# Gabisanth/MaximumAreaCoverageOptimization.jl

Hardware: AMD Instinct MI355X
Metric: MADS objective evals/sec (N UAVs × M fire cells), 1/2/4/8 MI355X (higher is better)
Workload: dtype f64

## Files before the change

maximumareacoverageoptimization.jl_amd/csrc/k_prep.h:

```cpp
#pragma once

#include <hip/hip_runtime.h>
#include <stdint.h>

#include "predicate.h"
#include "k_common.h"

#pragma clang fp contract(off)

namespace mac {


struct PenArgs {
    const double* rmax;
    const double* prev;
    const double* dlimT;
    const double* dlim;
    double tan_half_fov;
};

__device__ __forceinline__ double pen_threshold(const PenArgs& pa, int i)
{
    if (!pa.prev) return 0.0;
    return pa.dlimT ? pa.dlimT[i] : dlim_threshold(pa.dlim[i]);
}

__device__ __forceinline__ double pen_term(double x2, double y2, double R2, int i, int N,
                                           const PenArgs& pa, double T3)
{
    if (pa.prev) {
        const double x1 = pa.prev[i], y1 = pa.prev[N + i], z1 = pa.prev[2 * N + i] / pa.tan_half_fov;
        const double z2 = R2 / pa.tan_half_fov;
        const double ddx = x1 - x2, ddy = y1 - y2, ddz = z1 - z2;
        const double s = ddx * ddx + ddy * ddy + ddz * ddz;
        if (s > T3) return -1.0;
    }
    return pa.rmax ? __builtin_fabs(R2 - pa.rmax[i]) : 0.0;
}

__host__ __device__ __forceinline__ bool diag_rejects(double v, double b, double p, int q,
                                                      double tan_half_fov, double T3)
{
    bool all = true;
#pragma unroll
    for (int sg = 0; sg < 2; ++sg) {
        const double c = sg == 0 ? v + b : v - b;
        double d;
        if (q < 2) {
            d = p - c;
        } else {
            const double z1 = p / tan_half_fov, z2 = c / tan_half_fov;
            d = z1 - z2;
        }
        const double sq = d * d;
        all = all && sq > T3;
    }
    return all;
}


__host__ __device__ __forceinline__ uint64_t splitmix_at(uint64_t state, uint64_t idx)
{
    uint64_t z = state + idx * 0x9E3779B97F4A7C15ull;
    z = (z ^ (z >> 30)) * 0xBF58476D1CE4E5B9ull;
    z = (z ^ (z >> 27)) * 0x94D049BB133111EBull;
    return z ^ (z >> 31);
}

__host__ __device__ __forceinline__ double splitmix_uniform_at(uint64_t state, uint64_t idx)
{
    return (double)(splitmix_at(state, idx) >> 11) * (1.0 / 9007199254740992.0);
}

__host__ __device__ __forceinline__ double ltmads_entry(uint64_t state, int64_t n, int64_t b,
                                                        int64_t r, int64_t c)
{
    if (r < c) return 0.0;
    if (r == c) return (splitmix_uniform_at(state, (uint64_t)r + 1) < 0.5 ? -1.0 : 1.0) * (double)b;
    const int64_t lo = -b + 1, span = 2 * b - 1;
    const double u = splitmix_uniform_at(state, (uint64_t)(n + 1 + r * (r - 1) / 2 + c));
    return (double)(lo + (int64_t)__builtin_floor(u * (double)span));
}

struct MadsState {
    double f;
    int64_t it;
    int ell;
    int skip;
    unsigned long long feas;
    int64_t skipped;
    int64_t succ;
};

struct CandSrc {
    const double* cands;
    int ldc;
    const uint32_t* keysP;
    const float* keysT;
    int ldk;
    const double* xinc;
    const int* rp;
    const int* cp;
    uint64_t state;
    int64_t b;
    int k0;
    int np;
    const MadsState* mst;
    const int16_t* ltri;
    double delta;
    int route_five;
    __device__ __forceinline__ bool resolve(bool any_poll = false)
    {
        if (!mst) return true;
        const int e = mst->ell;
        if (e < 0 || (!any_poll && mst->skip)) return false;
        b = (int64_t)1 << e;
        return true;
    }
    __host__ __device__ __forceinline__ int polled(int N) const { return np ? np : 3 * N; }
    __device__ __forceinline__ double entry(int n, int r, int c) const
    {
        if (ltri) return r < c ? 0.0 : delta * (double)ltri[(int64_t)r * (r + 1) / 2 + c];
        return ltmads_entry(state, n, b, r, c);
    }
    __device__ __forceinline__ double get_full(int kl, int v, int N) const
    {
        if (cands) return cands[(int64_t)kl * ldc + v];
        const int n = 3 * N;
        const int k = kl + k0;
        const int kk = k < n ? k : k - n;
        const double d = entry(n, rp[v], cp[kk]);
        return k < n ? xinc[v] + d : xinc[v] - d;
    }
    __device__ __forceinline__ double get(int kl, int v, int N) const
    {
        if (cands) return cands[(int64_t)kl * ldc + v];
        const int n = polled(N);
        const int k = kl + k0;
        const int kk = k < n ? k : k - n;
        const bool held = v >= n;
// ... 40 lines not shown
    float* keysT;
    int ldk;
    double4* pd;
    uint8_t* dead8;
    MadsState* mst_w;
    unsigned long long* feas;
    int* lreset;
    const uint8_t* mask8;
};

template <int NC, class Cand>
__device__ __forceinline__ uint32_t prep_masked(const uint8_t* mask8, int K, Cand cand)
{
    uint32_t m = 0u;
    if (mask8) {
#pragma unroll
        for (int c = 0; c < NC; ++c) {
            const int k = cand(c);
            if (k < K && mask8[k] == 0) m |= 1u << c;
        }
    }
    return m;
}

constexpr int kPrepCX = 6;

constexpr uint32_t kKeyEsc = 0x200u << 22;
__device__ __forceinline__ bool key_int(double v, double b, double lim, int& d)
{
    const double f = v - b;
    if (!(f >= -lim && f <= lim)) return false;
    d = (int)f;
    return (double)d == f && __builtin_bit_cast(uint64_t, b + (double)d) == __builtin_bit_cast(uint64_t, v);
}
__device__ __forceinline__ uint32_t key_pack(int dx, int dy, int dr)
{
    return ((uint32_t)dx & 0x7FFu) | (((uint32_t)dy & 0x7FFu) << 11) | (((uint32_t)dr & 0x3FFu) << 22);
}
__device__ __forceinline__ void key_unpack(uint32_t p, float& x, float& y, float& r)
{
    x = (float)((int)(p << 21) >> 21);
    y = (float)((int)(p << 10) >> 21);
    r = (float)((int)p >> 22);
}

__device__ __forceinline__ bool partial_range(double a, double b, double m, double g0, double invS,
                                              int n, int& lo, int& hi)
{
    const double ulo = (a - g0) * invS;
    const double uhi = (b - g0) * invS;
    const double err = (m + __builtin_fabs(g0)) * invS * 1e-14 + 1e-9;
    const double flo = __builtin_floor(ulo - err);
    const double fhi = __builtin_floor(uhi + err);
    if (!(flo == flo) || !(fhi == fhi)) { lo = 0; hi = n - 1; return true; }
    if (fhi < 0.0 || flo > (double)(n - 1)) return false;
    lo = flo < 0.0 ? 0 : (int)flo;
    hi = fhi > (double)(n - 1) ? n - 1 : (int)fhi;
    return true;
}

__host__ __device__ inline int range_shift(int n)
{
    int s = 0;
    while (((n - 1) >> s) > 0xFFFE) ++s;
    return s;
}
__device__ __forceinline__ uint32_t range_pack(bool any, int lo, int hi, int s)
{
    return any ? (uint32_t)(lo >> s) | ((uint32_t)(hi >> s) << 16) : 0xFFFFu;
}
__device__ __forceinline__ void range_unpack(uint32_t lo16, uint32_t hi16, int s, int n, int& lo, int& hi)
{
    lo = (int)(lo16 << s);
    hi = min((int)(((hi16 + 1) << s) - 1), n - 1);
}

#ifdef MAC_DIAG
__device__ uint64_t g_diag_prep[64 * 16];
#define MAC_PREP_STAMP_T(q, t) if (threadIdx.x == (t) && cw < 64 && (q) < 16) g_diag_prep[16 * cw + (q)] = __builtin_amdgcn_s_memrealtime()
#else
#define MAC_PREP_STAMP_T(q, t)
#endif
#define MAC_PREP_STAMP(q) MAC_PREP_STAMP_T(q, 0)

__device__ __forceinline__ void lds_barrier()
{
    asm volatile("s_waitcnt lgkmcnt(0)\n\ts_barrier" ::: "memory");
}

template <int PC>
struct PrepLds {
    double term[PC][kPrepU + 2];
    int wbad[kPrepU / kWave][PC];
    uint32_t wbadm[kPrepU / kWave];
    int wrej[kPrepU / kWave];
    double dred[kPrepU / kWave][4];
};

template <bool kMat, int PC>
__device__ __forceinline__ void prep_block(const PrepArgs& a, int cw, unsigned char* lds)
{
    constexpr int NC = PC;
    PrepLds<NC>& L = *reinterpret_cast<PrepLds<NC>*>(lds);
    auto& term = L.term;
    auto& wbad = L.wbad;
    auto& wbadm = L.wbadm;
    auto& wrej = L.wrej;
    auto& dred = L.dred;
    const int N = a.N, K = a.K;
    const int u = threadIdx.x, lane = u & (kWave - 1), wid = u / kWave;
    const int k0 = cw * PC;
    const int np = a.src.polled(N);
    auto cand = [&](int c) { return a.pair ? (c < 4 ? 4 * cw + c : np + 4 * cw + c - 4) : k0 + c; };
    const bool obj = a.vp != nullptr;
    const PenArgs& pa = a.pa;
    MAC_PREP_STAMP(0);
    double acc = 0.0;
    bool bad = false;
    uint32_t mdead = 0u;
    if constexpr (!kMat) mdead = prep_masked<NC>(obj ? a.mask8 : nullptr, K, cand);
    const bool masked = !kMat && a.mask8 != nullptr;
    const bool excl = obj && (pa.prev || masked) && (a.prec || a.pd) && a.skip_failed && N <= kPrepU;
    double dmx = -__builtin_inf(), dmy = -__builtin_inf(), dmr = -__builtin_inf();
    double dml = -__builtin_inf();
    uint32_t dead = 0u;
    for (int ib = 0; ib < N; ib += kPrepU) {
        const int nb = min(kPrepU, N - ib);
        const int i = ib + u;
        const bool iv = u < nb;
        const int ii = min(i, N - 1);
        double v[NC][3];
        if (!kMat && PC == 8 && a.pair) {
#pragma unroll
            for (int c = 0; c < 4; ++c) {
                const int col = 4 * cw + c;
#pragma unroll
                for (int q = 0; q < 3; ++q) {
                    const int vv = q * N + ii;
                    if (q == 2 && 2 * N >= np) {
                        v[c][q] = v[c + 4][q] = a.src.xinc[vv];
                        continue;
                    }
                    const double d = a.src.entry(np, a.src.rp[vv], a.src.cp[col]);
                    v[c][q] = a.src.xinc[vv] + d;
                    v[c + 4][q] = a.src.xinc[vv] - d;
                }
            }
        } else {
#pragma unroll
            for (int c = 0; c < NC; ++c) {
                const int k = min(cand(c), K - 1);
#pragma unroll
                for (int q = 0; q < 3; ++q) {
                    if constexpr (kMat) v[c][q] = a.src.cands[(int64_t)k * a.src.ldc + q * N + ii];
                    else v[c][q] = a.src.get(k, q * N + ii, N);
                }
            }
        }
        double base[3] = {0.0, 0.0, 0.0};
        if (a.keysP) {
#pragma unroll
            for (int q = 0; q < 3; ++q) {
                if constexpr (kMat) base[q] = a.src.cands[q * N + ii];
                else base[q] = a.src.get(0, q * N + ii, N);
            }
        }
// ... 122 lines not shown
        }
        if ((a.prec || a.keysP) && iv) {
            double xa = __builtin_inf(), xb = -__builtin_inf(), ya = __builtin_inf(), yb = -__builtin_inf();
            double xm = 0.0, ym = 0.0, est = 0.0;
            bool any = false;
#pragma unroll
            for (int c = 0; c < NC; ++c) {
                if (!a.prec) break;
                const double x = v[c][0], y = v[c][1], r = v[c][2];
                if (cand(c) < K && !((dead >> c) & 1u) && r > 0.0 && __builtin_isfinite(x) &&
                    __builtin_isfinite(y)) {
                    any = true;
                    xa = fmin(xa, x - r);
                    xb = fmax(xb, x + r);
                    ya = fmin(ya, y - r);
                    yb = fmax(yb, y + r);
                    xm = fmax(xm, __builtin_fabs(x) + r);
                    ym = fmax(ym, __builtin_fabs(y) + r);
                    const double e = 2.0 * r * a.g.invS + 1.0;
                    est += e * e;
                }
            }
            bool kb = false;
            if (a.keysP) {
                uint32_t pk[NC];
#pragma unroll
                for (int c = 0; c < NC; ++c) {
                    int dx = 0, dy = 0, dr = 0;
                    const bool packs = key_int(v[c][0], base[0], 1023.0, dx) &&
                                       key_int(v[c][1], base[1], 1023.0, dy) &&
                                       key_int(v[c][2], base[2], 511.0, dr);
                    pk[c] = packs ? key_pack(dx, dy, dr) : kKeyEsc;
                    if (!packs) {
#pragma unroll
                        for (int q = 0; q < 3; ++q) {
                            const float f = (float)(v[c][q] - base[q]);
                            kb |= !((dead >> c) & 1u) && __builtin_bit_cast(uint64_t, base[q] + (double)f) != __builtin_bit_cast(uint64_t, v[c][q]);
                            a.keysT[(int64_t)(q * N + i) * a.ldk + cand(c)] = f;
                        }
                    }
                }
                uint32_t* const krow = a.keysP + (int64_t)i * a.ldk;
#pragma unroll
                for (int h = 0; h < PC / 4; ++h)
                    *reinterpret_cast<uint4*>(krow + cand(4 * h)) =
                        make_uint4(pk[4 * h], pk[4 * h + 1], pk[4 * h + 2], pk[4 * h + 3]);
            }
            if (a.prec) {
                int x0 = 0, x1 = -1, y0 = 0, y1 = -1;
                any = any && partial_range(xa, xb, xm, a.g.gx0, a.g.invS, a.g.nTx, x0, x1) &&
                      partial_range(ya, yb, ym, a.g.gy0, a.g.invS, a.g.nTy, y0, y1);
                a.prec[(int64_t)cw * N + i] =
                    make_int4((int)range_pack(any, x0, x1, range_shift(a.g.nTx)),
                              (int)range_pack(any, y0, y1, range_shift(a.g.nTy)),
                              __builtin_bit_cast(int, (float)est), kb ? 1 : 0);
            }
        }
        MAC_PREP_STAMP(3 + 3 * (ib / kPrepU));
        if (obj && ib + kPrepU < N) lds_barrier();
    }
    if (obj && u < NC && cand(u) < K) {
        a.vp[cand(u)] = bad ? __builtin_inf() : acc * a.penalty;
        if (a.dead8) a.dead8[cand(u)] = excl && bad ? 1 : 0;
    }
    if (obj && a.feas && wid == 0) {
        const uint64_t ok = __ballot(u < NC && cand(u) < K && !bad);
        if (lane == 0 && ok) atomicAdd(a.feas, (unsigned long long)__popcll(ok));
    }
    if (a.pd) {
        lds_barrier();
        if (u == 0) {
            double4 m = make_double4(dred[0][0], dred[0][1], dred[0][2], dred[0][3]);
            for (int q = 1; q < kPrepU / kWave; ++q) {
                m.x = fmax(m.x, dred[q][0]);
                m.y = fmax(m.y, dred[q][1]);
                m.z = fmax(m.z, dred[q][2]);
                m.w = fmax(m.w, dred[q][3]);
            }
            a.pd[cw] = m;
        }
    }
}

template <bool kGen>
__device__ __forceinline__ void prep_block_x(const PrepArgs& a, int cw, unsigned char* lds)
{
    constexpr int PC = kPrepCX, NC = kGen ? kPrepCX : kPrepCX + 1, NW = kPrepU / kWave;
    PrepLds<kPrepCX + 1>& L = *reinterpret_cast<PrepLds<kPrepCX + 1>*>(lds);
    auto& term = L.term;
    auto& wbad = L.wbad;
    auto& wbadm = L.wbadm;
    auto& wrej = L.wrej;
    auto& dred = L.dred;
    const int N = a.N, K = a.K;
    const int u = threadIdx.x, lane = u & (kWave - 1), wid = u / kWave;
    const bool fw = wid == NW;
    const int k0 = cw * PC;
    const int n3 = 3 * N;
    auto cand = [&](int c) {
        if constexpr (kGen) return c < 3 ? 3 * cw + c : n3 + 3 * cw + c - 3;
        else return c < PC ? k0 + c : a.xbase + cw;
    };
    const bool obj = a.vp != nullptr;
    const PenArgs& pa = a.pa;
    uint32_t mdead = 0u;
    if constexpr (kGen) mdead = prep_masked<NC>(obj ? a.mask8 : nullptr, K, cand);
    const bool masked = kGen && a.mask8 != nullptr;
    const bool excl = obj && (pa.prev || masked) && a.skip_failed;
    const bool iv = !fw && u < N;
    const int ii = min(u, N - 1);
    MAC_PREP_STAMP(0);
    double v[NC][3];
    double base[3] = {0.0, 0.0, 0.0};
    if (!fw) {
        if constexpr (kGen) {
#pragma unroll
            for (int q = 0; q < 3; ++q) {
                const int vv = q * N + ii;
                const int rv = a.src.rp[vv];
                const double xv = a.src.xinc[vv];
#pragma unroll
                for (int c = 0; c < 3; ++c) {
                    const double d = a.src.entry(n3, rv, a.src.cp[3 * cw + c]);
                    v[c][q] = xv + d;
                    v[c + 3][q] = xv - d;
                }
                base[q] = xv + a.src.entry(n3, rv, a.src.cp[0]);
            }
        } else {
#pragma unroll
            for (int c = 0; c < NC; ++c) {
                const int k = min(cand(c), K - 1);
#pragma unroll
                for (int q = 0; q < 3; ++q) v[c][q] = a.src.cands[(int64_t)k * a.src.ldc + q * N + ii];
            }
#pragma unroll
            for (int q = 0; q < 3; ++q) base[q] = a.src.cands[q * N + ii];
        }
        if (obj) {
            const double x1 = pa.prev ? pa.prev[ii] : 0.0, y1 = pa.prev ? pa.prev[N + ii] : 0.0;
            const double z1 = pa.prev ? pa.prev[2 * N + ii] / pa.tan_half_fov : 0.0;
            const double rm = pa.rmax ? pa.rmax[ii] : 0.0;
            const double T3 = pen_threshold(pa, ii);
            uint32_t wdead = 0u;
#pragma unroll
            for (int c = 0; c < NC; ++c) {
                const double R2 = v[c][2];
                double t = pa.rmax ? __builtin_fabs(R2 - rm) : 0.0;
                if (pa.prev) {
                    const double z2 = R2 / pa.tan_half_fov;
                    const double ddx = x1 - v[c][0], ddy = y1 - v[c][1], ddz = z1 - z2;
                    const double sq = ddx * ddx + ddy * ddy + ddz * ddz;
                    if (sq > T3) t = -1.0;
                }
                term[c][u] = t;
                const uint64_t neg = __ballot(iv && t < 0.0);
                if (lane == 0) wbad[wid][c] = neg != 0;
                wdead |= (neg != 0 ? 1u : 0u) << c;
            }
            if (lane == 0) wbadm[wid] = wdead;
            if (a.mst_w) {
                bool rej = true;
                if (iv) {
                    const double bb = (double)a.src.b;
                    rej = diag_rejects(a.src.xinc[ii], bb, x1, 0, pa.tan_half_fov, T3) &&
                          diag_rejects(a.src.xinc[N + ii], bb, y1, 1, pa.tan_half_fov, T3) &&
                          diag_rejects(a.src.xinc[2 * N + ii], bb, pa.prev[2 * N + ii], 2, pa.tan_half_fov, T3);
                }
                const uint64_t keep = __ballot(!rej);
                if (lane == 0) wrej[wid] = keep == 0;
            }
        }
    }
    MAC_PREP_STAMP(1);
    uint32_t dead = 0u;
    if (obj) {
        lds_barrier();
        if (excl) {
            dead = mdead;
#pragma unroll
            for (int w = 0; w < NW; ++w) dead |= wbadm[w];
            if (a.mst_w) {
                bool rej = true;
#pragma unroll
                for (int w = 0; w < NW; ++w) rej = rej && wrej[w] != 0;
                if (cw == 0 && u == 0) a.mst_w->skip = rej ? 1 : 0;
                if (rej) return;
            }
        }
    }
    MAC_PREP_STAMP(2);
    if (fw) {
        bool bad = false;
        double acc = 0.0;
        if (obj && lane < NC) {
#pragma unroll
            for (int w = 0; w < NW; ++w) bad |= wbad[w][lane] != 0;
            if constexpr (kGen) bad |= ((mdead >> lane) & 1u) != 0;
            if (!bad) {
                constexpr int kB = 6;
                const double2* row2 = reinterpret_cast<const double2*>(&term[lane][0]);
                const int nfull = N / (2 * kB);
                __builtin_amdgcn_s_setprio(3);
                auto batch = [&](double2 (&buf)[kB], int bt) {
                    const int at = (bt < nfull ? bt : nfull - 1) * kB;
#pragma unroll
                    for (int j = 0; j < kB; ++j) buf[j] = row2[at + j];
                };
                auto add = [&](const double2 (&buf)[kB]) {
#pragma unroll
                    for (int j = 0; j < kB; ++j) {
                        acc += buf[j].x;
                        acc += buf[j].y;
                    }
                };
                if (nfull > 0) {
                    double2 A[kB], B[kB];
                    batch(A, 0);
#pragma unroll 1
                    for (int bt = 0; bt < nfull; bt += 2) {
                        batch(B, bt + 1);
                        __builtin_amdgcn_sched_barrier(0);
                        add(A);
                        if (bt + 1 >= nfull) break;
                        batch(A, bt + 2);
                        __builtin_amdgcn_sched_barrier(0);
                        add(B);
                    }
                }
                for (int q = nfull * 2 * kB; q < N; ++q) acc += term[lane][q];
                __builtin_amdgcn_s_setprio(0);
            }
            MAC_PREP_STAMP_T(3, kPrepU);
            if (cand(lane) < K) {
                a.vp[cand(lane)] = bad ? __builtin_inf() : acc * a.penalty;
                if (a.dead8) a.dead8[cand(lane)] = excl && bad ? 1 : 0;
            }
        }
        if (obj && a.feas) {
            const uint64_t ok = __ballot(lane < NC && cand(lane) < K && !bad);
            if (lane == 0 && ok) atomicAdd(a.feas, (unsigned long long)__popcll(ok));
        }
    } else {
        double dmx = -__builtin_inf(), dmy = -__builtin_inf(), dmr = -__builtin_inf(), dml = -__builtin_inf();
        uint32_t pk[NC];
        bool kb = false;
#pragma unroll
        for (int c = 0; c < NC; ++c) {
            const double x = v[c][0], y = v[c][1], r = v[c][2];
            int dx = 0, dy = 0, dr = 0;
            const bool packs = key_int(x, base[0], 1023.0, dx) && key_int(y, base[1], 1023.0, dy) &&
                               key_int(r, base[2], 511.0, dr);
            pk[c] = packs ? key_pack(dx, dy, dr) : kKeyEsc;
            if (!packs && iv && cand(c) < K) {
#pragma unroll
                for (int q = 0; q < 3; ++q) {
                    const float f = (float)(v[c][q] - base[q]);
                    if constexpr (kGen)
                        kb |= !((dead >> c) & 1u) &&
                              __builtin_bit_cast(uint64_t, base[q] + (double)f) != __builtin_bit_cast(uint64_t, v[c][q]);
                    a.keysT[(int64_t)(q * N + u) * a.ldk + cand(c)] = f;
                }
            }
            if (a.pd && iv && cand(c) < K && !((dead >> c) & 1u) && r > 0.0 && __builtin_isfinite(x) &&
                __builtin_isfinite(y)) {
                double ex = __builtin_fabs(x - base[0]), ey = __builtin_fabs(y - base[1]), er = r - base[2];
                double el = base[2] - r;
                if (!(ex <= kDblMax)) ex = __builtin_inf();
                if (!(ey <= kDblMax)) ey = __builtin_inf();
                if (!(er == er)) er = __builtin_inf();
                if (!(el == el)) el = __builtin_inf();
                dmx = fmax(dmx, ex);
                dmy = fmax(dmy, ey);
                dmr = fmax(dmr, er);
                dml = fmax(dml, el);
            }
        }
        if (iv) {
            uint32_t* const krow = a.keysP + (int64_t)u * a.ldk;
            if constexpr (kGen) {
#pragma unroll
                for (int c = 0; c < NC; ++c) krow[cand(c)] = pk[c];
            } else {
                static_assert(PC % 2 == 0, "an even candidate count");
#pragma unroll
                for (int h = 0; h < PC / 2; ++h)
                    *reinterpret_cast<uint2*>(krow + k0 + 2 * h) = make_uint2(pk[2 * h], pk[2 * h + 1]);
                if (cand(PC) < K) krow[cand(PC)] = pk[PC];
            }
        }
        if (kGen && a.prec && iv) {
            double xa = __builtin_inf(), xb = -__builtin_inf(), ya = __builtin_inf(), yb = -__builtin_inf();
            double xm = 0.0, ym = 0.0, est = 0.0;
            bool any = false;
#pragma unroll
            for (int c = 0; c < NC; ++c) {
                const double x = v[c][0], y = v[c][1], r = v[c][2];
                if (cand(c) < K && !((dead >> c) & 1u) && r > 0.0 && __builtin_isfinite(x) &&
                    __builtin_isfinite(y)) {
                    any = true;
                    xa = fmin(xa, x - r);
                    xb = fmax(xb, x + r);
                    ya = fmin(ya, y - r);
                    yb = fmax(yb, y + r);
                    xm = fmax(xm, __builtin_fabs(x) + r);
                    ym = fmax(ym, __builtin_fabs(y) + r);
                    const double e = 2.0 * r * a.g.invS + 1.0;
                    est += e * e;
                }
            }
            int x0 = 0, x1 = -1, y0 = 0, y1 = -1;
            any = any && partial_range(xa, xb, xm, a.g.gx0, a.g.invS, a.g.nTx, x0, x1) &&
                  partial_range(ya, yb, ym, a.g.gy0, a.g.invS, a.g.nTy, y0, y1);
            a.prec[(int64_t)cw * N + u] =
                make_int4((int)range_pack(any, x0, x1, range_shift(a.g.nTx)),
                          (int)range_pack(any, y0, y1, range_shift(a.g.nTy)),
                          __builtin_bit_cast(int, (float)est), kb ? 1 : 0);
        }
        if (a.pd) {
#pragma unroll
            for (int o = 32; o >= 1; o >>= 1) {
                dmx = fmax(dmx, __shfl_xor(dmx, o, kWave));
                dmy = fmax(dmy, __shfl_xor(dmy, o, kWave));
                dmr = fmax(dmr, __shfl_xor(dmr, o, kWave));
                dml = fmax(dml, __shfl_xor(dml, o, kWave));
            }
            if (lane == 0) {
                dred[wid][0] = dmx;
                dred[wid][1] = dmy;
                dred[wid][2] = dmr;
                dred[wid][3] = dml;
            }
        }
    }
    if (a.pd) {
        lds_barrier();
        if (u == 0) {
            double4 m = make_double4(dred[0][0], dred[0][1], dred[0][2], dred[0][3]);
            for (int q = 1; q < NW; ++q) {
                m.x = fmax(m.x, dred[q][0]);
                m.y = fmax(m.y, dred[q][1]);
                m.z = fmax(m.z, dred[q][2]);
                m.w = fmax(m.w, dred[q][3]);
            }
            a.pd[cw] = m;
        }
    }
}

template <int PC, bool kX = false, bool kGen = false>
__device__ __forceinline__ void prep_body(uint64_t* ts, PrepArgs& a)
{
    ts_begin(ts);
    if (a.lreset && blockIdx.x == 0 && threadIdx.x == 0) *a.lreset = 0;
    if (!a.src.resolve(true)) {
        ts_end(ts);
        return;
    }
    const int per = (int)((gridDim.x + 7) / 8), b = (int)blockIdx.x;
    const int cw = (int)(gridDim.x % 8) == 0 ? (b % 8) * per + b / 8 : b;
    __shared__ __attribute__((aligned(16))) unsigned char lds[sizeof(PrepLds<kX ? PC + 1 : PC>)];
    if constexpr (kX) {
        prep_block_x<kGen>(a, cw, lds);
    } else if (a.src.cands) {
        prep_block<true, PC>(a, cw, lds);
    } else {
        prep_block<false, PC>(a, cw, lds);
    }
    ts_end(ts);
}

__global__ __launch_bounds__(kPrepU) __attribute__((amdgpu_waves_per_eu(4))) void prep_kernel(uint64_t* ts, PrepArgs a)
{
    prep_body<kPrepC>(ts, a);
}

template <bool kGen>
__global__ __launch_bounds__(kPrepU + kWave) __attribute__((amdgpu_waves_per_eu(6))) void prep_x_kernel(uint64_t* ts, PrepArgs a)
{
    prep_body<kPrepCX, true, kGen>(ts, a);
}

__global__ void disk_prep_kernel(CandSrc src, int N, int K, DiskRec* __restrict__ disks)
{
    const int64_t t = (int64_t)blockIdx.x * blockDim.x + threadIdx.x;
    if (t >= (int64_t)N * K) return;
    const int k = (int)(t / N), i = (int)(t % N);
    disks[t] = make_disk(src.get(k, i, N), src.get(k, N + i, N), src.get(k, 2 * N + i, N));
}

}
```

maximumareacoverageoptimization.jl_amd/csrc/maxcover.hip:

```cpp
#include <hip/hip_runtime.h>
#include <hip/hip_ext.h>
#include <dlfcn.h>
#include <sched.h>
#include <linux/futex.h>
#include <sys/syscall.h>
#include <unistd.h>
#include <hipcub/hipcub.hpp>
#include <immintrin.h>

#include <algorithm>
#include <chrono>
#include <atomic>
#include <cmath>
#include <cstdio>
#include <cstdlib>
#include <cstring>
#include <deque>
#include <mutex>
#include <new>
#include <string>
#include <type_traits>
#include <thread>
#include <vector>

// ... 81 lines not shown
        cap = 0;
    }
    template <class T>
    T* as() const { return (T*)p; }
};

struct PinnedBuf {
    void* p = nullptr;
    size_t cap = 0;
    void reserve(size_t b, unsigned flags = hipHostMallocDefault)
    {
        if (b <= cap) return;
        if (p && t_defer_free)
            t_defer_free->push_back({p, true});
        else if (p)
            HCK(hipHostFree(p));
        p = nullptr;
        cap = 0;
        HCK(hipHostMalloc(&p, b, flags));
        cap = b;
    }
    void release()
    {
        if (p) (void)hipHostFree(p);
        p = nullptr;
        cap = 0;
    }
};

struct Lane {
    hipStream_t stream = nullptr;
    hipStream_t last = nullptr;
    hipEvent_t done = nullptr;
    DevBuf cands, disks, partial, area, obj, best, rmax, prev, dlim, region, mode, nbr,
        ncount, dlist, spart, vp, xinc, perm, ucount, umap, keysT, lane4, lanexp, rows, nboxT,
        cnt, dlimraw, finblk, finarrive, c32, p32, qual, nboxU, ncountU, orjobs;
    std::vector<double> h_dlim;
    PinnedBuf h_stage;
    PinnedBuf h_io;
    PinnedBuf h_dc;
    int* d_dc = nullptr;
    int dc_hist[8] = {};
    PinnedBuf h_cl;
    uint64_t* d_cl = nullptr;
    uint64_t cl_seq = 0;
    DevBuf cpart, carrive, ctot;
    DevBuf clv;
    DevBuf bdpart, bdarrive, bdout;
    DevBuf cmask, cbest;
    DevBuf prec, cost;
    int um_hist[8] = {};
    int walk_hist[8] = {};
    DevBuf pd, dead8, frows, fwhint, fwlist, fwcount, fwsxy, fwsw;
    int last_chain = 0;
};

struct RcclUid {
    char internal[128];
};
struct RcclApi {
    void* lib = nullptr;
    int (*get_unique_id)(RcclUid*) = nullptr;
    int (*comm_init_rank)(void**, int, RcclUid, int) = nullptr;
    int (*all_gather)(const void*, void*, size_t, int, void*, hipStream_t) = nullptr;
    int (*comm_destroy)(void*) = nullptr;
    const char* (*error_string)(int) = nullptr;
};

struct mac_ctx {
    int device = 0;
    int cus = 256;
    std::mutex mu;
    bool host_stats = false;
    double hs_t[4] = {0, 0, 0, 0};
    int64_t hs_n = 0;
    RcclApi* rccl = nullptr;
    void* comm = nullptr;
    int comm_rank = 0, comm_world = 0;
    void* d_xrec = nullptr;
    std::mutex xmu;
    PinnedBuf h_xrec;
    void* d_xrec2 = nullptr;
    std::atomic<uint64_t> fused_bad{0};
    std::atomic<bool> route_seeded{false};
    std::mutex cl_mu;
    std::deque<struct ClReq*> cl_q;
    std::atomic<int> cl_busy{0};
    std::atomic<int> cl_active{0};
    int cl_taken = 0;
    std::atomic<uint32_t> cl_gen{0};
    std::atomic<int> cl_genw[64] = {};
    int64_t cl_batches = 0, cl_reqs = 0;
    std::atomic<int64_t> cl_phase_ns[4] = {};
    std::atomic<int64_t> cl_req_ns[5] = {};
    std::atomic<int64_t> cl_led{0};
    std::vector<Lane*> lanes_free;
    std::vector<Lane*> lanes_all;
    hipStream_t setup_stream = nullptr;
    static constexpr int kMirrorSlots = 64;
    PinnedBuf h_mirror;
    uint64_t* d_mirror = nullptr;
    const void* mirror_key[kMirrorSlots] = {};
    uint64_t mirror_want[kMirrorSlots] = {};
    uint64_t mirror_used[kMirrorSlots] = {};
    uint64_t mirror_seq = 0, mirror_clock = 0;
    uint64_t* doorbell = nullptr;
    uint64_t armed = 0, fired = 0;
    std::vector<uint64_t> voided;
    std::vector<std::pair<hipStream_t, uint64_t>> armed_on;
    std::vector<std::pair<void*, bool>> deferred;

    int algo = MAC_ALGO_AUTO;
    int shared_mode = MAC_SHARED_AUTO;
    int chain = MAC_CHAIN_AUTO;
    bool profile = false;
    struct Prof { int64_t a, na, b, nb; int64_t K; const int* mode; int algo;
                  int64_t c = -1, nc = 0, f = -1, nf = 0;
                  int64_t role[MAC_PROF_ROLES][2] = {{-1, 0}, {-1, 0}, {-1, 0}, {-1, 0}, {-1, 0},
                                                     {-1, 0}, {-1, 0}, {-1, 0}, {-1, 0}, {-1, 0}}; };
    std::vector<Prof> prof;
    DevBuf stamps;
    int64_t stamp_cap = 0, stamp_used = 0;
    int storage = MAC_STORE_F64;
    int tile_ppt = 4;

    int64_t M = 0;
    bool has_points = false;
    DevBuf x, y, w;
    DevBuf xys, ws, perm, off;
    Grid grid{};
    int64_t nTiles = 1;
    bool w_uniform = false;
    std::atomic<bool> cl_bar{false};
    double w0 = 0.0;
    DevBuf keys_in, keys_out, idx_in, tmp, bbox, flags_s, flags_o, keep, sel_count, cx, cy, cw,
        cidx, circ, cdisk;
    int n_regions = 0;
    double reg_w_high = NAN;
    double h_boxes[4 * kRegionsMax];
    DevBuf rboxes, rcount, ritems, rpart, rout;
};

static void set_device(mac_ctx* ctx) { HCK(hipSetDevice(ctx->device)); }

static void free_deferred(mac_ctx* ctx)
{
    std::vector<std::pair<void*, bool>> v;
    {
        std::lock_guard<std::mutex> lk(ctx->mu);
        v.swap(ctx->deferred);
    }
    for (auto& d : v) (void)(d.second ? hipHostFree(d.first) : hipFree(d.first));
}

static Lane* acquire_lane(mac_ctx* ctx, hipStream_t want, bool ordered = false)
{
    {
        std::lock_guard<std::mutex> lk(ctx->mu);
        if (ordered) {
            for (size_t i = 0; i < ctx->lanes_free.size(); ++i) {
                Lane* l = ctx->lanes_free[i];
                if (l->last == want) {
                    ctx->lanes_free.erase(ctx->lanes_free.begin() + (long)i);
                    return l;
                }
            }
// ... 423 lines not shown
            pr.mask8 = d_mask8;
            pr.lreset = L->fwcount.as<int>();
            uint64_t* tsk = take_ts(nprep, ts_c, ts_nc);
            using hclk = std::chrono::steady_clock;
            hclk::time_point h1, h2, h3;
            if (ctx->host_stats) h1 = hclk::now();
            if (xk && gen_x)
                hipLaunchKernelGGL(prep_x_kernel<true>, dim3((unsigned)nprep), dim3(kPrepU + kWave), 0, s, tsk, pr);
            else if (xk)
                hipLaunchKernelGGL(prep_x_kernel<false>, dim3((unsigned)nprep), dim3(kPrepU + kWave), 0, s, tsk, pr);
            else hipLaunchKernelGGL(prep_kernel, dim3((unsigned)nprep), dim3(kPrepU), 0, s, tsk, pr);
            HCK(hipGetLastError());
            if (ctx->host_stats) h2 = hclk::now();
            FwArgs fa{};
            fa.src = src;
            fa.src.keysP = pr.keysP;
            fa.src.keysT = pr.keysT;
            fa.src.ldk = ldk;
            fa.N = N;
            fa.K = K;
            fa.g = ctx->grid;
            fa.dead = pr.dead8;
            fa.pd = pr.pd;
            fa.npd = nprep;
            fa.xy = ctx->xys.as<double2>();
            fa.w = ctx->ws.as<double>();
            fa.off = ctx->off.as<int32_t>();
            fa.counts = counts;
            fa.crow = L->frows.as<unsigned>();
            fa.frow = L->frows.as<double>();
            fa.ldk = ldk;
            fa.hint = L->fwhint.as<int>();
            fa.sh = FwShared{L->fwcount.as<int>(), L->fwlist.as<int4>(), L->fwsxy.as<double2>(),
                             L->fwsw.as<double>()};
            const F2Shared f2s{fa.src, L->fwcount.as<int>(), L->fwlist.as<int4>(), L->fwsxy.as<double2>(),
                               L->fwsw.as<double>(), fa.dead};
            const unsigned nfw = 8 * (unsigned)((N + 7) / 8);
            uint64_t* tsw = take_ts(nfw, ts_w, ts_nw);
            ts_a = ts_w;
            ts_na = ts_nw;
            const bool mat = src.cands != nullptr;
            const auto fiw_kern = counts ? (mat ? fiw_kernel<true, true> : fiw_kernel<true, false>)
                                         : (mat ? fiw_kernel<false, true> : fiw_kernel<false, false>);
            hipLaunchKernelGGL(fiw_kern, dim3(nfw), dim3(kFwThreads), 0, s, tsw, fa);
            HCK(hipGetLastError());
            if (ctx->host_stats) h3 = hclk::now();
            const unsigned nfin = 8 * (unsigned)((K + 8 * kF2C - 1) / (8 * kF2C));
            FinBest fb{};
            if (d_best) {
                L->finblk.reserve(2 * sizeof(unsigned long long) * nfin);
                if (L->finarrive.grow(sizeof(unsigned)))
                    HCK(hipMemsetAsync(L->finarrive.p, 0, L->finarrive.cap, s));
                if (fb_mads) fb = *fb_mads;
                fb.best = d_best;
                fb.mirror = d_mirror;
                fb.seq = mirror_seq;
                fb.idx_base = idx_base;
                fb.blk = L->finblk.as<unsigned long long>();
                fb.arrive = L->finarrive.as<unsigned>();
                fb.hint = L->fwhint.as<int>();
                fb.hint_host = L->d_dc + 8;
                fb.nhint = kFwHints;
                fb.feas = d_mirror ? d_feas : nullptr;
            }
            uint64_t* tsf = take_ts(nfin, ts_f, ts_nf);
            const bool xy = fb.np != 0 && !mat;
            const auto fin2_kern =
                counts ? (mat ? fin2_kernel<true, true> : xy ? fin2_kernel<true, false, true> : fin2_kernel<true, false>)
                       : (mat ? fin2_kernel<false, true> : xy ? fin2_kernel<false, false, true> : fin2_kernel<false, false>);
            hipLaunchKernelGGL(fin2_kern, dim3(nfin), dim3(kF2Threads), 0, s,
                               counts ? L->frows.as<unsigned>() : nullptr, counts ? nullptr : L->frows.as<double>(),
                               ldk, N, K, ctx->w0, d_vp, d_area, d_obj, fb, f2s, tsf);
            HCK(hipGetLastError());
            if (ctx->host_stats) {
                const auto h4 = hclk::now();
                std::lock_guard<std::mutex> lk(ctx->mu);
                ctx->hs_t[0] += std::chrono::duration<double>(h1 - t_poll_entry).count();
                ctx->hs_t[1] += std::chrono::duration<double>(h2 - h1).count();
                ctx->hs_t[2] += std::chrono::duration<double>(h3 - h2).count();
                ctx->hs_t[3] += std::chrono::duration<double>(h4 - h3).count();
                ++ctx->hs_n;
            }
            L->last_chain = 2;
            prof_end();
            return;
        }
    }
    if (poll_possible) L->last_chain = 1;
    int nrec = nchain;

    if ((d_obj || poll_possible) && K > 0) {
        const bool gx5 = gen_x && poll_possible && want_keys;
        nrec = gx5 ? N : nchain;
        PrepArgs pr{};
        pr.src = src;
        pr.N = N;
        pr.K = K;
        pr.pa = pa;
        pr.penalty = penalty;
        pr.vp = d_vp;
        pr.nchain = nrec;
        pr.skip_failed = d_area ? 0 : 1;
        pr.pair = pair ? 1 : 0;
        pr.g = ctx->grid;
        pr.feas = d_feas;
        pr.mask8 = d_mask8;
        pr.mst_w = fb_mads && poll_possible && d_obj && d_prev && !d_area && N <= kPrepU ? fb_mads->st
                                                                                           : nullptr;
        if (poll_possible) {
            L->prec.reserve(sizeof(int4) * (size_t)nrec * N);
            pr.prec = L->prec.as<int4>();
        }
        if (want_keys) {
            const int ldk = keys_ld(K);
            L->keysT.reserve(sizeof(float) * (size_t)4 * N * ldk);
            pr.keysP = L->keysT.as<uint32_t>();
            pr.keysT = L->keysT.as<float>() + (size_t)N * ldk;
            pr.ldk = ldk;
            isrc.keysP = pr.keysP;
            isrc.keysT = pr.keysT;
            isrc.ldk = ldk;
        }
        uint64_t* tsk = poll_possible ? take_ts(nrec, ts_c, ts_nc) : nullptr;
        if (gx5) hipLaunchKernelGGL(prep_x_kernel<true>, dim3((unsigned)nrec), dim3(kPrepU + kWave), 0, s, tsk, pr);
        else hipLaunchKernelGGL(prep_kernel, dim3((unsigned)nchain), dim3(kPrepU), 0, s, tsk, pr);
        HCK(hipGetLastError());
    }

    if (N == 0 || M == 0) {
        L->partial.reserve(sizeof(double) * (size_t)K);
        HCK(hipMemsetAsync(L->partial.p, 0, sizeof(double) * (size_t)K, s));
    } else if (!tiled) {
        L->disks.reserve(sizeof(DiskRec) * (size_t)N * K);
        hipLaunchKernelGGL(disk_prep_kernel, dim3(grid1d((int64_t)N * K, 256)), dim3(256), 0, s,
                           src, N, K, L->disks.as<DiskRec>());
        HCK(hipGetLastError());
        constexpr int KB = 4, PPT = 4;
        const int64_t per_pass = (int64_t)kBlock * PPT;
        int64_t nblk = std::max<int64_t>(1, (M + per_pass - 1) / per_pass);
        const int kgroups = (K + KB - 1) / KB;
        const int64_t want = std::max<int64_t>(1, (int64_t)(8 * ctx->cus) / kgroups);
        nblk = std::min(nblk, want);
        int64_t chunk = (M + nblk - 1) / nblk;
        chunk = ((chunk + per_pass - 1) / per_pass) * per_pass;
        nblk = std::max<int64_t>(1, (M + chunk - 1) / chunk);
        n_other = (int)nblk;
        L->partial.reserve(sizeof(double) * (size_t)K * nblk);
        uint64_t* ts = take_ts(nblk * kgroups, ts_a, ts_na);
        hipLaunchKernelGGL((coverage_scan_kernel<KB, PPT>), dim3((unsigned)nblk, (unsigned)kgroups),
                           dim3(kBlock), 0, s, ts, ctx->xys.as<double2>(), ctx->ws.as<double>(), M,
                           L->disks.as<DiskRec>(), N, K, chunk, L->partial.as<double>());
        HCK(hipGetLastError());
    } else {
        L->disks.reserve(sizeof(DiskRec) * (size_t)N * K);
        L->umap.reserve(sizeof(int) * (size_t)N * K);
        L->ucount.reserve(sizeof(int) * (size_t)N);
        if (poll_possible) {
            L->lane4.reserve(sizeof(float4) * (size_t)N * K);
            L->lanexp.reserve(sizeof(float) * (size_t)N * K);
            L->rows.reserve(sizeof(int2) * (size_t)N * (kRowInfo + 1));
        }
        counts = poll_possible && ctx->w_uniform ? 1 : 0;
        n_other = G;
        const DiskRec* d_urec = L->disks.as<DiskRec>();
        const int* d_map = L->umap.as<int>();
        if (!poll_possible) {
            const int64_t nk = (int64_t)N * K;
            hipLaunchKernelGGL(disk_index_identity_kernel, dim3(grid1d(nk, 256)), dim3(256), 0, s,
                               src, N, K, L->disks.as<DiskRec>(), L->umap.as<int>());
// ... 496 lines not shown
                            hipMemcpyDeviceToHost) != hipSuccess)
        return MAC_E_HIP;
    return MAC_OK;
}

int32_t mac_diag_fiw_read(uint64_t* out, int64_t n)
{
    if (n > (int64_t)(16 * 65536)) n = 16 * 65536;
    if (hipMemcpyFromSymbol(out, HIP_SYMBOL(g_diag_fiw), sizeof(uint64_t) * n, 0,
                            hipMemcpyDeviceToHost) != hipSuccess)
        return MAC_E_HIP;
    return MAC_OK;
}

int32_t mac_diag_f2_read(uint64_t* out, int64_t n)
{
    if (n > (int64_t)(8 * 4096)) n = 8 * 4096;
    if (hipMemcpyFromSymbol(out, HIP_SYMBOL(g_diag_f2), sizeof(uint64_t) * n, 0,
                            hipMemcpyDeviceToHost) != hipSuccess)
        return MAC_E_HIP;
    return MAC_OK;
}

int32_t mac_diag_prep_read(uint64_t* out, int64_t n)
{
    if (n > 64 * 16) n = 64 * 16;
    if (hipMemcpyFromSymbol(out, HIP_SYMBOL(g_diag_prep), sizeof(uint64_t) * n, 0,
                            hipMemcpyDeviceToHost) != hipSuccess)
        return MAC_E_HIP;
    return MAC_OK;
}

int32_t mac_diag_bits_read(uint64_t* out, int64_t n)
{
    if (n > 256 * 16) n = 256 * 16;
    if (hipMemcpyFromSymbol(out, HIP_SYMBOL(g_diag_bits), sizeof(uint64_t) * n, 0,
                            hipMemcpyDeviceToHost) != hipSuccess)
        return MAC_E_HIP;
    return MAC_OK;
}

int32_t mac_diag_or_read(uint64_t* out, int64_t n)
{
    if (n > 1024 * 16) n = 1024 * 16;
    if (hipMemcpyFromSymbol(out, HIP_SYMBOL(g_diag_or), sizeof(uint64_t) * n, 0,
                            hipMemcpyDeviceToHost) != hipSuccess)
        return MAC_E_HIP;
    return MAC_OK;
}

int32_t mac_diag_stamps(mac_ctx* ctx, uint64_t* out, int64_t n, int64_t* used)
{
    if (!ctx) return MAC_E_INVAL;
    if (hipDeviceSynchronize() != hipSuccess) return MAC_E_HIP;
    std::lock_guard<std::mutex> lk(ctx->mu);
    *used = ctx->stamp_used;
    n = std::min<int64_t>(n, 2 * ctx->stamp_used);
    if (n > 0 && hipMemcpy(out, ctx->stamps.p, sizeof(uint64_t) * n, hipMemcpyDeviceToHost) != hipSuccess)
        return MAC_E_HIP;
    return MAC_OK;
}

int32_t mac_diag_read(uint64_t* out, int64_t n)
{
    if (n > (int64_t)(4 * kDiagMax)) n = 4 * kDiagMax;
    if (hipMemcpyFromSymbol(out, HIP_SYMBOL(g_diag), sizeof(uint64_t) * n, 0, hipMemcpyDeviceToHost) != hipSuccess)
        return MAC_E_HIP;
    return MAC_OK;
}
#endif

int32_t mac_diag_grid(double xmn, double xmx, double ymn, double ymx, int64_t M, int32_t tile_points,
                      double* out)
{
    if (!out || tile_points < 1) return MAC_E_INVAL;
    const Grid g = choose_grid(xmn, xmx, ymn, ymx, M, tile_points);
    out[0] = g.S;
    out[1] = g.invS;
    out[2] = (double)g.nTx;
    out[3] = (double)g.nTy;
    return MAC_OK;
}

int32_t mac_diag_tiles(double c, double r, double g0, double invS, int32_t n, int32_t* out)
{
    if (!out || n < 1) return MAC_E_INVAL;
    int lo = -1, hi = -1;
    out[0] = tile_of(c, g0, invS, n);
    out[1] = tile_span(c, r, g0, invS, n, lo, hi) ? 1 : 0;
    out[2] = lo;
    out[3] = hi;
    return MAC_OK;
}

const char* mac_last_error(void) { return g_last_error.c_str(); }

const char* mac_version(void) { return "maxcover 0.1.0 gfx950"; }

double mac_cover_threshold(double r) { return cover_threshold(r); }

int32_t mac_profile_read(mac_ctx* ctx, double* kernel_ms, int64_t* launches,
                         int64_t* candidates, int32_t* last_algo, int32_t reset)
{
    ABI_BEGIN
    if (!ctx) return fail(MAC_E_INVAL, "null context");
    set_device(ctx);
    HCK(hipDeviceSynchronize());
    std::lock_guard<std::mutex> lk(ctx->mu);
    std::vector<uint64_t> st((size_t)(2 * ctx->stamp_used));
    if (!st.empty())
        HCK(hipMemcpy(st.data(), ctx->stamps.p, sizeof(uint64_t) * st.size(), hipMemcpyDeviceToHost));
    double ms = 0.0;
    int64_t n = 0, kc = 0;
    int algo = 0;
    auto span_ms = [&](int64_t base, int64_t nwg) {
        uint64_t t0 = ~(uint64_t)0, t1 = 0;
        for (int64_t q = base; q < base + nwg; ++q) {
            t0 = std::min(t0, st[(size_t)(2 * q)]);
            t1 = std::max(t1, st[(size_t)(2 * q + 1)]);
        }
        return t1 > t0 ? (double)(t1 - t0) / kRealtimeHz * 1e3 : 0.0;
    };
    for (auto& p : ctx->prof) {
        algo = p.algo;
        int64_t a = p.a, na = p.na;
        if (p.mode) {
            int m = 0;
            HCK(hipMemcpy(&m, p.mode, sizeof(int), hipMemcpyDeviceToHost));
            algo = m == kModePoll ? MAC_ALGO_POLL : MAC_ALGO_TILED;
            if (m == kModePoll) {
                a = p.b;
                na = p.nb;
            }
        }
        if (a < 0) continue;
        ms += span_ms(a, na);
        ++n;
        kc += p.K;
    }
    if (kernel_ms) *kernel_ms = ms;
    if (launches) *launches = n;
    if (candidates) *candidates = kc;
    if (last_algo) *last_algo = algo;
    if (reset) {
        ctx->prof.clear();
        if (ctx->stamp_used) HCK(hipMemset(ctx->stamps.p, 0, sizeof(uint64_t) * 2 * ctx->stamp_used));
        ctx->stamp_used = 0;
    }
    return MAC_OK;
    ABI_END
}

int32_t mac_profile_split(mac_ctx* ctx, double* prep_ms, double* walk_ms, double* gap_ms,
                          int64_t* polls)
{
    ABI_BEGIN
    if (!ctx) return fail(MAC_E_INVAL, "null context");
    set_device(ctx);
    HCK(hipDeviceSynchronize());
    std::lock_guard<std::mutex> lk(ctx->mu);
    std::vector<uint64_t> st((size_t)(2 * ctx->stamp_used));
    if (!st.empty())
        HCK(hipMemcpy(st.data(), ctx->stamps.p, sizeof(uint64_t) * st.size(), hipMemcpyDeviceToHost));
    double a1 = 0.0, a2 = 0.0, gap = 0.0;
    int64_t n = 0;
    for (auto& p : ctx->prof) {
// ... 2572 lines not shown
```

Before: 44.82 million.

## Add fast-path feasibility test and integer bound reduction in prep_block_x

For the non-generated candidate path, the prep kernel replaces the per-candidate division by tan_half_fov with a multiply by a wave-uniform reciprocal. It keeps an error-bounded margin check and falls back to the exact division only when some lane is near the threshold. The displacement-bound reduction now uses integer maxima from the packed deltas with DPP wave reductions. It refetches candidates and runs the old double path only if a lane cannot be packed. Loads go through scalar-base plus lane-offset addressing, and a diagnostic API exposes prep outputs; the exchange is extra code complexity and a rarely used fallback branch.

```diff
diff --git a/maximumareacoverageoptimization.jl_amd/csrc/k_prep.h b/maximumareacoverageoptimization.jl_amd/csrc/k_prep.h
--- a/maximumareacoverageoptimization.jl_amd/csrc/k_prep.h
+++ b/maximumareacoverageoptimization.jl_amd/csrc/k_prep.h
@@ -56,6 +56,23 @@
         all = all && sq > T3;
     }
     return all;
+}
+
+__host__ __device__ __forceinline__ bool cons3_inv_ok(double inv)
+{
+    const double ai = __builtin_fabs(inv);
+    return ai >= 0x1p-1000 && ai <= 0x1p1000;
+}
+__host__ __device__ __forceinline__ bool cons3_fast(double ddx, double ddy, double z1, double z2f,
+                                                    double T3, bool& fail)
+{
+    const double ddz = z1 - z2f;
+    const double sq = ddx * ddx + ddy * ddy + ddz * ddz;
+    const double Z = __builtin_fabs(z1) + __builtin_fabs(z2f);
+    const double m = 0x1p-46 * (Z * Z + sq);
+    const double gap = __builtin_fabs(sq - T3);
+    fail = sq > T3;
+    return gap > m && gap < __builtin_inf() && m >= 0x1p-500;
 }
 
 
@@ -262,6 +279,11 @@
 #define MAC_PREP_STAMP_T(q, t)
 #endif
 #define MAC_PREP_STAMP(q) MAC_PREP_STAMP_T(q, 0)
+#ifdef MAC_DIAG
+#define MAC_PREP_LANDED(q) do { asm volatile("s_waitcnt vmcnt(0)" ::: "memory"); MAC_PREP_STAMP(q); } while (0)
+#else
+#define MAC_PREP_LANDED(q)
+#endif
 
 __device__ __forceinline__ void lds_barrier()
 {
@@ -550,6 +572,31 @@
     }
 }
 
+template <class T>
+__device__ __forceinline__ T ld_lane(const T* base, uint32_t off8)
+{
+    typedef const char __attribute__((address_space(1))) * gbytes;
+    typedef const T __attribute__((address_space(1))) * gvalue;
+    gbytes b = (gbytes)base;
+    asm("" : "+s"(b));
+    return *(gvalue)(b + off8);
+}
+
+template <int kCtrl, int kRows>
+__device__ __forceinline__ int dpp_max_step(int v)
+{
+    return max(v, __builtin_amdgcn_update_dpp(v, v, kCtrl, kRows, 0xF, false));
+}
+__device__ __forceinline__ int wave_max_lane63(int v)
+{
+    v = dpp_max_step<0xB1, 0xF>(v);
+    v = dpp_max_step<0x4E, 0xF>(v);
+    v = dpp_max_step<0x141, 0xF>(v);
+    v = dpp_max_step<0x140, 0xF>(v);
+    v = dpp_max_step<0x142, 0xA>(v);
+    return dpp_max_step<0x143, 0xC>(v);
+}
+
 template <bool kGen>
 __device__ __forceinline__ void prep_block_x(const PrepArgs& a, int cw, unsigned char* lds)
 {
@@ -580,6 +627,13 @@
     MAC_PREP_STAMP(0);
     double v[NC][3];
     double base[3] = {0.0, 0.0, 0.0};
+    constexpr bool kFast = !kGen;
+    const uint32_t lo8 = (uint32_t)ii * 8u;
+    auto refetch = [&](int c, int q) -> double {
+        int k = c < 0 ? 0 : min(cand(c), K - 1);
+        asm("" : "+s"(k));
+        return ld_lane(a.src.cands + (int64_t)k * a.src.ldc + q * N, lo8);
+    };
     if (!fw) {
         if constexpr (kGen) {
 #pragma unroll
@@ -599,32 +653,62 @@
 #pragma unroll
             for (int c = 0; c < NC; ++c) {
                 const int k = min(cand(c), K - 1);
-#pragma unroll
-                for (int q = 0; q < 3; ++q) v[c][q] = a.src.cands[(int64_t)k * a.src.ldc + q * N + ii];
-            }
-#pragma unroll
-            for (int q = 0; q < 3; ++q) base[q] = a.src.cands[q * N + ii];
-        }
+                const double* cb = a.src.cands + (int64_t)k * a.src.ldc;
+#pragma unroll
+                for (int q = 0; q < 3; ++q) v[c][q] = ld_lane(cb + q * N, lo8);
+            }
+#pragma unroll
+            for (int q = 0; q < 3; ++q) base[q] = ld_lane(a.src.cands + q * N, lo8);
+        }
+        MAC_PREP_LANDED(4);
         if (obj) {
             const double x1 = pa.prev ? pa.prev[ii] : 0.0, y1 = pa.prev ? pa.prev[N + ii] : 0.0;
             const double z1 = pa.prev ? pa.prev[2 * N + ii] / pa.tan_half_fov : 0.0;
             const double rm = pa.rmax ? pa.rmax[ii] : 0.0;
             const double T3 = pen_threshold(pa, ii);
             uint32_t wdead = 0u;
-#pragma unroll
-            for (int c = 0; c < NC; ++c) {
-                const double R2 = v[c][2];
-                double t = pa.rmax ? __builtin_fabs(R2 - rm) : 0.0;
-                if (pa.prev) {
-                    const double z2 = R2 / pa.tan_half_fov;
-                    const double ddx = x1 - v[c][0], ddy = y1 - v[c][1], ddz = z1 - z2;
-                    const double sq = ddx * ddx + ddy * ddy + ddz * ddz;
-                    if (sq > T3) t = -1.0;
-                }
-                term[c][u] = t;
-                const uint64_t neg = __ballot(iv && t < 0.0);
-                if (lane == 0) wbad[wid][c] = neg != 0;
-                wdead |= (neg != 0 ? 1u : 0u) << c;
+            if constexpr (kFast) {
+                const uint64_t invb = __builtin_bit_cast(uint64_t, pa.prev ? 1.0 / pa.tan_half_fov : 0.0);
+                uint32_t invlo, invhi;
+                asm("v_readfirstlane_b32 %0, %1" : "=s"(invlo) : "v"((uint32_t)invb));
+                asm("v_readfirstlane_b32 %0, %1" : "=s"(invhi) : "v"((uint32_t)(invb >> 32)));
+                const double inv = __builtin_bit_cast(double, ((uint64_t)invhi << 32) | invlo);
+                const bool inv_bad = pa.prev && !cons3_inv_ok(inv);
+#pragma unroll
+                for (int c = 0; c < NC; ++c) {
+                    const double R2 = v[c][2];
+                    bool fail = false;
+                    if (pa.prev) {
+                        const double ddx = x1 - v[c][0], ddy = y1 - v[c][1];
+                        const bool near = !cons3_fast(ddx, ddy, z1, R2 * inv, T3, fail) || inv_bad;
+                        if (__ballot(iv && near) != 0) {
+                            const double z2 = R2 / pa.tan_half_fov;
+                            const double ddz = z1 - z2;
+                            const double sq = ddx * ddx + ddy * ddy + ddz * ddz;
+                            fail = sq > T3;
+                        }
+                    }
+                    term[c][u] = fail ? -1.0 : pa.rmax ? __builtin_fabs(R2 - rm) : 0.0;
+                    const uint64_t neg = __ballot(iv && fail);
+                    if (lane == 0) wbad[wid][c] = neg != 0;
+                    wdead |= (neg != 0 ? 1u : 0u) << c;
+                }
+            } else {
+#pragma unroll
+                for (int c = 0; c < NC; ++c) {
+                    const double R2 = v[c][2];
+                    double t = pa.rmax ? __builtin_fabs(R2 - rm) : 0.0;
+                    if (pa.prev) {
+                        const double z2 = R2 / pa.tan_half_fov;
+                        const double ddx = x1 - v[c][0], ddy = y1 - v[c][1], ddz = z1 - z2;
+                        const double sq = ddx * ddx + ddy * ddy + ddz * ddz;
+                        if (sq > T3) t = -1.0;
+                    }
+                    term[c][u] = t;
+                    const uint64_t neg = __ballot(iv && t < 0.0);
+                    if (lane == 0) wbad[wid][c] = neg != 0;
+                    wdead |= (neg != 0 ? 1u : 0u) << c;
+                }
             }
             if (lane == 0) wbadm[wid] = wdead;
             if (a.mst_w) {
@@ -710,6 +794,9 @@
             if (lane == 0 && ok) atomicAdd(a.feas, (unsigned long long)__popcll(ok));
         }
     } else {
+        constexpr int kNoD = -1024;
+        int ix = -1, iy = -1, ir = kNoD, il = kNoD;
+        bool esc = false;
         double dmx = -__builtin_inf(), dmy = -__builtin_inf(), dmr = -__builtin_inf(), dml = -__builtin_inf();
         uint32_t pk[NC];
         bool kb = false;
@@ -730,8 +817,19 @@
                     a.keysT[(int64_t)(q * N + u) * a.ldk + cand(c)] = f;
                 }
             }
-            if (a.pd && iv && cand(c) < K && !((dead >> c) & 1u) && r > 0.0 && __builtin_isfinite(x) &&
-                __builtin_isfinite(y)) {
+            if constexpr (kFast) {
+                if (a.pd) {
+                    const bool in = iv && cand(c) < K && !((dead >> c) & 1u);
+                    esc |= in && !packs;
+                    if (in && packs && r > 0.0) {
+                        ix = max(ix, max(dx, -dx));
+                        iy = max(iy, max(dy, -dy));
+                        ir = max(ir, dr);
+                        il = max(il, -dr);
+                    }
+                }
+            } else if (a.pd && iv && cand(c) < K && !((dead >> c) & 1u) && r > 0.0 && __builtin_isfinite(x) &&
+                       __builtin_isfinite(y)) {
                 double ex = __builtin_fabs(x - base[0]), ey = __builtin_fabs(y - base[1]), er = r - base[2];
                 double el = base[2] - r;
                 if (!(ex <= kDblMax)) ex = __builtin_inf();
@@ -745,7 +843,9 @@
             }
         }
         if (iv) {
-            uint32_t* const krow = a.keysP + (int64_t)u * a.ldk;
+            uint32_t* const krow =
+                kFast ? reinterpret_cast<uint32_t*>(reinterpret_cast<char*>(a.keysP) + (uint32_t)u * (uint32_t)a.ldk * 4u)
+                      : a.keysP + (int64_t)u * a.ldk;
             if constexpr (kGen) {
 #pragma unroll
                 for (int c = 0; c < NC; ++c) krow[cand(c)] = pk[c];
@@ -786,23 +886,68 @@
                           __builtin_bit_cast(int, (float)est), kb ? 1 : 0);
         }
         if (a.pd) {
-#pragma unroll
-            for (int o = 32; o >= 1; o >>= 1) {
-                dmx = fmax(dmx, __shfl_xor(dmx, o, kWave));
-                dmy = fmax(dmy, __shfl_xor(dmy, o, kWave));
-                dmr = fmax(dmr, __shfl_xor(dmr, o, kWave));
-                dml = fmax(dml, __shfl_xor(dml, o, kWave));
-            }
-            if (lane == 0) {
-                dred[wid][0] = dmx;
-                dred[wid][1] = dmy;
-                dred[wid][2] = dmr;
-                dred[wid][3] = dml;
-            }
-        }
-    }
+            bool ints = false;
+            if constexpr (kFast) {
+                ints = __ballot(esc) == 0;
+                if (ints) {
+                    ix = wave_max_lane63(ix);
+                    iy = wave_max_lane63(iy);
+                    ir = wave_max_lane63(ir);
+                    il = wave_max_lane63(il);
+                    if (lane == kWave - 1) {
+                        dred[wid][0] = ix < 0 ? -__builtin_inf() : (double)ix;
+                        dred[wid][1] = iy < 0 ? -__builtin_inf() : (double)iy;
+                        dred[wid][2] = ir == kNoD ? -__builtin_inf() : (double)ir;
+                        dred[wid][3] = il == kNoD ? -__builtin_inf() : (double)il;
+                    }
+                } else {
+                    double b0 = 0.0, b1 = 0.0, b2 = 0.0;
+#pragma unroll 1
+                    for (int c = -1; c < NC; ++c) {
+                        const double x = refetch(c, 0), y = refetch(c, 1), r = refetch(c, 2);
+                        if (c < 0) {
+                            b0 = x;
+                            b1 = y;
+                            b2 = r;
+                            continue;
+                        }
+                        if (iv && cand(c) < K && !((dead >> c) & 1u) && r > 0.0 && __builtin_isfinite(x) &&
+                            __builtin_isfinite(y)) {
+                            double ex = __builtin_fabs(x - b0), ey = __builtin_fabs(y - b1), er = r - b2;
+                            double el = b2 - r;
+                            if (!(ex <= kDblMax)) ex = __builtin_inf();
+                            if (!(ey <= kDblMax)) ey = __builtin_inf();
+                            if (!(er == er)) er = __builtin_inf();
+                            if (!(el == el)) el = __builtin_inf();
+                            dmx = fmax(dmx, ex);
+                            dmy = fmax(dmy, ey);
+                            dmr = fmax(dmr, er);
+                            dml = fmax(dml, el);
+                        }
+                    }
+                }
+            }
+            if (!ints) {
+#pragma unroll
+                for (int o = 32; o >= 1; o >>= 1) {
+                    dmx = fmax(dmx, __shfl_xor(dmx, o, kWave));
+                    dmy = fmax(dmy, __shfl_xor(dmy, o, kWave));
+                    dmr = fmax(dmr, __shfl_xor(dmr, o, kWave));
+                    dml = fmax(dml, __shfl_xor(dml, o, kWave));
+                }
+                if (lane == 0) {
+                    dred[wid][0] = dmx;
+                    dred[wid][1] = dmy;
+                    dred[wid][2] = dmr;
+                    dred[wid][3] = dml;
+                }
+            }
+        }
+    }
+    MAC_PREP_STAMP(5);
     if (a.pd) {
         lds_barrier();
+        MAC_PREP_STAMP(6);
         if (u == 0) {
             double4 m = make_double4(dred[0][0], dred[0][1], dred[0][2], dred[0][3]);
             for (int q = 1; q < NW; ++q) {
@@ -814,6 +959,7 @@
             a.pd[cw] = m;
         }
     }
+    MAC_PREP_STAMP(7);
 }
 
 template <int PC, bool kX = false, bool kGen = false>
diff --git a/maximumareacoverageoptimization.jl_amd/csrc/maxcover.hip b/maximumareacoverageoptimization.jl_amd/csrc/maxcover.hip
--- a/maximumareacoverageoptimization.jl_amd/csrc/maxcover.hip
+++ b/maximumareacoverageoptimization.jl_amd/csrc/maxcover.hip
@@ -187,6 +187,14 @@
     PinnedBuf h_xrec;
     void* d_xrec2 = nullptr;
     std::atomic<uint64_t> fused_bad{0};
+    struct PrepOut {
+        bool valid = false;
+        int N = 0, K = 0, npd = 0, ldk = 0;
+        const double4* pd = nullptr;
+        const uint32_t* keysP = nullptr;
+        const uint8_t* dead8 = nullptr;
+        const double* vp = nullptr;
+    } prep_out;
     std::atomic<bool> route_seeded{false};
     std::mutex cl_mu;
     std::deque<struct ClReq*> cl_q;
@@ -776,9 +784,17 @@
                 ++ctx->hs_n;
             }
             L->last_chain = 2;
+            {
+                std::lock_guard<std::mutex> lk(ctx->mu);
+                ctx->prep_out = {true, N, K, nprep, ldk, pr.pd, pr.keysP, pr.dead8, d_vp};
+            }
             prof_end();
             return;
         }
+    }
+    {
+        std::lock_guard<std::mutex> lk(ctx->mu);
+        ctx->prep_out.valid = false;
     }
     if (poll_possible) L->last_chain = 1;
     int nrec = nchain;
@@ -1441,6 +1457,48 @@
     return MAC_OK;
 }
 
+int32_t mac_diag_prep_out(mac_ctx* ctx, int64_t row, int64_t cap, double* bound4, uint32_t* keys,
+                          uint8_t* dead, double* vp, int32_t* flags, int64_t* K_out)
+{
+    ABI_BEGIN
+    if (!ctx || !bound4 || !keys || !dead || !vp || !flags || !K_out) return fail(MAC_E_INVAL, "null argument");
+    set_device(ctx);
+    HCK(hipDeviceSynchronize());
+    mac_ctx::PrepOut po;
+    {
+        std::lock_guard<std::mutex> lk(ctx->mu);
+        po = ctx->prep_out;
+    }
+    if (!po.valid) return fail(MAC_E_INVAL, "the last poll did not run the fused chain");
+    if (row < 0 || row >= po.N || cap < po.K) return fail(MAC_E_INVAL, "row or cap out of range");
+    std::vector<double4> pd((size_t)po.npd);
+    HCK(hipMemcpy(pd.data(), po.pd, sizeof(double4) * pd.size(), hipMemcpyDeviceToHost));
+    double4 m = pd[0];
+    for (size_t q = 1; q < pd.size(); ++q) {
+        m.x = std::fmax(m.x, pd[q].x);
+        m.y = std::fmax(m.y, pd[q].y);
+        m.z = std::fmax(m.z, pd[q].z);
+        m.w = std::fmax(m.w, pd[q].w);
+    }
+    bound4[0] = m.x;
+    bound4[1] = m.y;
+    bound4[2] = m.z;
+    bound4[3] = m.w;
+    HCK(hipMemcpy(keys, po.keysP + (size_t)row * po.ldk, sizeof(uint32_t) * (size_t)po.K, hipMemcpyDeviceToHost));
+    *flags = 0;
+    if (po.dead8) {
+        HCK(hipMemcpy(dead, po.dead8, (size_t)po.K, hipMemcpyDeviceToHost));
+        *flags |= 1;
+    }
+    if (po.vp) {
+        HCK(hipMemcpy(vp, po.vp, sizeof(double) * (size_t)po.K, hipMemcpyDeviceToHost));
+        *flags |= 2;
+    }
+    *K_out = po.K;
+    return MAC_OK;
+    ABI_END
+}
+
 int32_t mac_diag_tiles(double c, double r, double g0, double invS, int32_t n, int32_t* out)
 {
     if (!out || n < 1) return MAC_E_INVAL;
```

Result: no change. 45.18 million (median of 2 runs) (+0.8%).
